# Quantus-Network/qp-zk-circuits

Hardware: AMD Instinct MI355X
Metric: Wormhole proofs/sec (higher is better)
Workload: dtype u64

## Files before the change

qp-zk-circuits_amd/csrc/merkle_kernels_mx.hip:

```cpp
#define POSEIDON_GROUPED_SBOX 1
#include <hip/hip_runtime.h>
#include <vector>
#include "merkle.hpp"
#include "poseidon_mfma.hpp"
#include "prover_kernels.hpp"

using gl::u32;
using gl::u64;

namespace mx {
constexpr int WG = 512;
__constant__ u64 c_poseidon_rc[poseidon::ROUNDS * poseidon::WIDTH];
__device__ uint4 g_table[pmf::TABLE_BYTES / 16];
__device__ uint4 g_table_p2[pmf::TABLE_BYTES / 16];

#define MX_KERNEL __global__ void __launch_bounds__(WG) __attribute__((amdgpu_waves_per_eu(4, 4)))

struct PoseidonV1 {
    static __device__ __forceinline__ const uint4 *table() { return g_table; }
    static __device__ __forceinline__ void permute(u64 (&s)[12], const poseidon2::Params *, const unsigned char *lds) { pmf::permute(s, c_poseidon_rc, lds); }
};
struct Poseidon2QP {
    static __device__ __forceinline__ const uint4 *table() { return g_table_p2; }
    static __device__ __forceinline__ void permute(u64 (&s)[12], const poseidon2::Params *p2, const unsigned char *lds) { pmf::permute_p2qp(s, *p2, lds); }
};
template <class Perm>
__device__ __forceinline__ const unsigned char *table_to_lds() {
    extern __shared__ uint4 mx_lds[];
    const uint4 *t = Perm::table();
    for (int i = threadIdx.x; i < pmf::TABLE_BYTES / 16; i += WG) mx_lds[i] = t[i];
    __syncthreads();
    return (const unsigned char *)mx_lds;
}
__device__ __forceinline__ u32 ilog2_64(u64 x) { return 63u - (u32)__clzll((long long)x); }

template <class Perm>
MX_KERNEL leaf_hash_kernel(MerkleLeafArgs a, const poseidon2::Params *p2) {
    const unsigned char *lds = table_to_lds<Perm>();
    const u64 total = a.n_leaves * a.batch;
    u64 gj = blockIdx.x * (u64)WG + threadIdx.x;
    const bool live = gj < total;
    gj = live ? gj : total - 1;
    const u64 pr = gj >> ilog2_64(a.n_leaves), j = gj & (a.n_leaves - 1);
    a.src0 += pr * a.ps_src0; a.src1 += pr * a.ps_src1; a.digests += pr * a.ps_digests;
    const u32 W = a.ncols0 + a.ncols1;
    auto elem = [&](u32 c) -> u64 {
        return c < a.ncols0 ? a.src0[(u64)c * a.stride0 + j] : a.src1[(u64)(c - a.ncols0) * a.stride1 + j];
    };
    u64 s[12];
#pragma unroll
    for (int i = 0; i < 12; i++) s[i] = 0;
    for (u32 c = 0; c < W; c += 8) {
#pragma unroll
        for (int i = 0; i < 8; i++)
            if (c + i < W) s[i] = elem(c + i);
        Perm::permute(s, p2, lds);
    }
    if (live) {
        u64 *out = a.digests + j * 4;
#pragma unroll
        for (int i = 0; i < 4; i++) out[i] = s[i];
    }
}

template <class Perm>
MX_KERNEL node_kernel(const u64 *in, u64 *out, u64 n_out, u32 batch, u64 ps, u32 per_thread, const poseidon2::Params *p2) {
    const unsigned char *lds = table_to_lds<Perm>();
    const u64 total = n_out * batch;
    const u32 sh = ilog2_64(n_out);
    for (u32 k = 0; k < per_thread; k++) {
        u64 gi = ((u64)blockIdx.x * per_thread + k) * WG + threadIdx.x;
        const bool live = gi < total;
        gi = live ? gi : total - 1;
        const u64 pr = gi >> sh, i = gi & (n_out - 1);
        const ulonglong2 *p = reinterpret_cast<const ulonglong2 *>(in + pr * ps + i * 8);
        const ulonglong2 a = p[0], b = p[1], c = p[2], d = p[3];
        u64 s[12];
        s[0] = a.x; s[1] = a.y; s[2] = b.x; s[3] = b.y; s[4] = c.x; s[5] = c.y; s[6] = d.x; s[7] = d.y;
        s[8] = s[9] = s[10] = s[11] = 0;
        Perm::permute(s, p2, lds);
        if (live) {
            ulonglong2 *o = reinterpret_cast<ulonglong2 *>(out + pr * ps + i * 4);
            o[0] = make_ulonglong2(s[0], s[1]);
            o[1] = make_ulonglong2(s[2], s[3]);
        }
    }
}

template <class Perm>
MX_KERNEL pow_kernel(PowArgs a, const poseidon2::Params *p2) {
    const u32 chunk = blockIdx.x / a.batch, pr = (blockIdx.x % a.batch + chunk) % a.batch;
    const u64 first = (u64)chunk * WG;
    if (first >= a.count) return;
    const u64 base = a.bases[pr];
    if (base == ~0ull) return;
    __shared__ u32 s_leave;
    if (threadIdx.x == 0) s_leave = __hip_atomic_load(&a.results[pr], __ATOMIC_RELAXED, __HIP_MEMORY_SCOPE_AGENT) < base + first ? 1u : 0u;
    __syncthreads();
    if (s_leave) return;
    const unsigned char *lds = table_to_lds<Perm>();
    const u64 idx = first + threadIdx.x, nonce = base + idx;
    const u64 *st = a.states + 12 * (u64)pr;
    u64 s[12];
#pragma unroll
    for (int i = 0; i < 12; i++) s[i] = (i == (int)a.pos) ? nonce : st[i];
    Perm::permute(s, p2, lds);
    if (idx < a.count && (s[7] >> (64 - a.pow_bits)) == 0) atomicMin((unsigned long long *)&a.results[pr], (unsigned long long)nonce);
}

template <class Perm>
MX_KERNEL selftest_kernel(u64 *states, const poseidon2::Params *p2) {
    const unsigned char *lds = table_to_lds<Perm>();
    const u64 t = blockIdx.x * (u64)WG + threadIdx.x;
    u64 s[12];
#pragma unroll
    for (int i = 0; i < 12; i++) s[i] = states[t * 12 + i];
    Perm::permute(s, p2, lds);
#pragma unroll
    for (int i = 0; i < 12; i++) states[t * 12 + i] = s[i];
}
}

template <class Perm>
static hipError_t allow_table_in_lds() {
    hipError_t e = hipFuncSetAttribute((const void *)mx::leaf_hash_kernel<Perm>, hipFuncAttributeMaxDynamicSharedMemorySize, pmf::TABLE_BYTES);
    if (e == hipSuccess) e = hipFuncSetAttribute((const void *)mx::node_kernel<Perm>, hipFuncAttributeMaxDynamicSharedMemorySize, pmf::TABLE_BYTES);
    if (e == hipSuccess) e = hipFuncSetAttribute((const void *)mx::pow_kernel<Perm>, hipFuncAttributeMaxDynamicSharedMemorySize, pmf::TABLE_BYTES);
    return e;
}
template <class Perm, class HostPerm>
static hipError_t device_selftest(HostPerm host_perm, const poseidon2::Params *host_p2) {
    constexpr int N = 4 * mx::WG;
    std::vector<u64> in((size_t)N * 12), out((size_t)N * 12);
    u64 seed = 0x9E3779B97F4A7C15ull;
    for (int t = 0; t < N; t++)
        for (int i = 0; i < 12; i++) {
            seed = seed * 6364136223846793005ull + 1442695040888963407ull;
            u64 v = (seed ^ (seed >> 31)) % gl::P;
            if (t % 9 == 0) v = (i & 1) ? gl::P - 1 - (v & 3) : (v & 7);
            in[(size_t)t * 12 + i] = v;
        }
    u64 *d = nullptr; poseidon2::Params *dp = nullptr; hipStream_t st = nullptr;
    hipError_t e = hipMalloc((void **)&d, in.size() * 8);
    if (e == hipSuccess && host_p2) { e = hipMalloc((void **)&dp, sizeof *host_p2); if (e == hipSuccess) e = hipMemcpy(dp, host_p2, sizeof *host_p2, hipMemcpyHostToDevice); }
    if (e == hipSuccess) e = hipMemcpy(d, in.data(), in.size() * 8, hipMemcpyHostToDevice);
    if (e == hipSuccess) e = hipStreamCreateWithFlags(&st, hipStreamNonBlocking);
    if (e == hipSuccess) e = hipFuncSetAttribute((const void *)mx::selftest_kernel<Perm>, hipFuncAttributeMaxDynamicSharedMemorySize, pmf::TABLE_BYTES);
    if (e == hipSuccess) {
        hipLaunchKernelGGL(mx::selftest_kernel<Perm>, dim3(N / mx::WG), dim3(mx::WG), pmf::TABLE_BYTES, st, d, dp);
        e = hipGetLastError();
        if (e == hipSuccess) e = hipStreamSynchronize(st);
    }
    if (e == hipSuccess) e = hipMemcpy(out.data(), d, out.size() * 8, hipMemcpyDeviceToHost);
    if (e == hipSuccess)
        for (int t = 0; t < N && e == hipSuccess; t++) {
            u64 s[12];
            for (int i = 0; i < 12; i++) s[i] = in[(size_t)t * 12 + i];
            host_perm(s);
            for (int i = 0; i < 12; i++) if (s[i] != out[(size_t)t * 12 + i]) e = hipErrorAssert;
        }
    constexpr u64 NL = 1ull << 19, NN = NL / 2, POW_COUNT = 1ull << 18;
    constexpr u32 WCOLS = 5, POW_BITS = 11, POW_BATCH = 2;
    u64 *d_cols = nullptr, *d_dig = nullptr, *d_pow = nullptr;
    std::vector<u64> cols((size_t)WCOLS * NL), dig(4 * (NL + NN)), powbuf(12 * POW_BATCH + 2 * POW_BATCH);
    if (e == hipSuccess) {
        for (size_t i = 0; i < cols.size(); i++) { seed = seed * 6364136223846793005ull + 1442695040888963407ull; cols[i] = (seed ^ (seed >> 29)) % gl::P; }
        for (u32 b = 0; b < POW_BATCH; b++) {
            for (int i = 0; i < 12; i++) { seed = seed * 6364136223846793005ull + 1442695040888963407ull; powbuf[12 * b + i] = (seed ^ (seed >> 29)) % gl::P; }
            powbuf[12 * POW_BATCH + b] = 1000 * (b + 1);
            powbuf[12 * POW_BATCH + POW_BATCH + b] = ~0ull;
        }
        e = hipMalloc((void **)&d_cols, cols.size() * 8);
        if (e == hipSuccess) e = hipMalloc((void **)&d_dig, dig.size() * 8);
        if (e == hipSuccess) e = hipMalloc((void **)&d_pow, powbuf.size() * 8);
        if (e == hipSuccess) e = hipMemcpy(d_cols, cols.data(), cols.size() * 8, hipMemcpyHostToDevice);
        if (e == hipSuccess) e = hipMemcpy(d_pow, powbuf.data(), powbuf.size() * 8, hipMemcpyHostToDevice);
    }
    if (e == hipSuccess) {
        MerkleLeafArgs la{};
        la.src0 = d_cols; la.stride0 = NL; la.ncols0 = WCOLS; la.n_leaves = NL; la.digests = d_dig; la.batch = 1;
        hipLaunchKernelGGL(mx::leaf_hash_kernel<Perm>, dim3((unsigned)(NL / mx::WG)), dim3(mx::WG), pmf::TABLE_BYTES, st, la, dp);
        hipLaunchKernelGGL(mx::node_kernel<Perm>, dim3((unsigned)(NN / mx::WG)), dim3(mx::WG), pmf::TABLE_BYTES, st, d_dig, d_dig + 4 * NL, NN, 1u, (u64)0, 1u, dp);
        PowArgs pa{};
        pa.states = d_pow; pa.bases = d_pow + 12 * POW_BATCH; pa.results = d_pow + 12 * POW_BATCH + POW_BATCH;
        pa.pos = 3; pa.pow_bits = POW_BITS; pa.batch = POW_BATCH; pa.count = POW_COUNT;
        hipLaunchKernelGGL(mx::pow_kernel<Perm>, dim3((unsigned)(POW_COUNT / mx::WG * POW_BATCH)), dim3(mx::WG), pmf::TABLE_BYTES, st, pa, dp);
        e = hipGetLastError();
        if (e == hipSuccess) e = hipStreamSynchronize(st);
        if (e == hipSuccess) e = hipMemcpy(dig.data(), d_dig, dig.size() * 8, hipMemcpyDeviceToHost);
        if (e == hipSuccess) e = hipMemcpy(powbuf.data(), d_pow, powbuf.size() * 8, hipMemcpyDeviceToHost);
    }
    if (e == hipSuccess) {
        for (u64 w = 0; w < NL / 64 && e == hipSuccess; w++) {
            const u64 j = w * 64 + (w * 7) % 64;
            u64 s[12] = {0};
            for (u32 c = 0; c < WCOLS; c++) s[c] = cols[(size_t)c * NL + j];
            host_perm(s);
            for (int i = 0; i < 4; i++) if (s[i] != dig[4 * j + i]) e = hipErrorAssert;
        }
        for (u64 w = 0; w < NN / 64 && e == hipSuccess; w++) {
            const u64 i0 = w * 64 + (w * 11) % 64;
            u64 s[12] = {0};
            for (int i = 0; i < 8; i++) s[i] = dig[8 * i0 + i];
            host_perm(s);
            for (int i = 0; i < 4; i++) if (s[i] != dig[4 * NL + 4 * i0 + i]) e = hipErrorAssert;
        }
        for (u32 b = 0; b < POW_BATCH && e == hipSuccess; b++) {
            const u64 base = 1000 * (b + 1), got = powbuf[12 * POW_BATCH + POW_BATCH + b];
            u64 want = ~0ull;
            for (u64 k = 0; k < POW_COUNT && want == ~0ull; k++) {
                u64 s[12];
                for (int i = 0; i < 12; i++) s[i] = i == 3 ? base + k : powbuf[12 * b + i];
                host_perm(s);
                if ((s[7] >> (64 - POW_BITS)) == 0) want = base + k;
            }
            if (got != want) e = hipErrorAssert;
        }
    }
    if (d_cols) (void)hipFree(d_cols);
    if (d_dig) (void)hipFree(d_dig);
    if (d_pow) (void)hipFree(d_pow);
    if (st) (void)hipStreamDestroy(st);
    if (d) (void)hipFree(d);
    if (dp) (void)hipFree(dp);
    return e;
}
hipError_t merkle_mx_upload_constants(const u64 *rc360) {
    std::vector<unsigned char> tab(pmf::TABLE_BYTES);
    if (!pmf::build_tables(rc360, tab.data()) || !pmf::host_selfcheck(rc360, tab.data(), 64)) return hipErrorInvalidValue;
    hipError_t e = hipMemcpyToSymbol(HIP_SYMBOL(mx::c_poseidon_rc), rc360, sizeof(u64) * poseidon::ROUNDS * poseidon::WIDTH);
    if (e != hipSuccess) return e;
    e = hipMemcpyToSymbol(HIP_SYMBOL(mx::g_table), tab.data(), pmf::TABLE_BYTES);
    if (e == hipSuccess) e = allow_table_in_lds<mx::PoseidonV1>();
    return e != hipSuccess ? e : device_selftest<mx::PoseidonV1>([&](u64 (&s)[12]) { poseidon::permute(s, rc360); }, nullptr);
}
hipError_t merkle_upload_p2_tables(const poseidon2::Params &qp) {
    std::vector<unsigned char> tab(pmf::TABLE_BYTES);
    if (!pmf::build_tables_p2(qp, tab.data()) || !pmf::host_selfcheck_p2(qp, tab.data(), 64)) return hipErrorInvalidValue;
    hipError_t e = hipMemcpyToSymbol(HIP_SYMBOL(mx::g_table_p2), tab.data(), pmf::TABLE_BYTES);
    if (e == hipSuccess) e = allow_table_in_lds<mx::Poseidon2QP>();
    return e != hipSuccess ? e : device_selftest<mx::Poseidon2QP>([&](u64 (&s)[12]) { poseidon2::permute(s, qp); }, &qp);
}
hipError_t merkle_mx_leaves(const MerkleLeafArgs &a, u64 total, const HasherDev &h, hipStream_t st) {
    const u64 blocks = (total + mx::WG - 1) / mx::WG;
    if (blocks > 0x7FFFFFFFull) return hipErrorInvalidValue;
    if (h.kind == hasher::POSEIDON2) hipLaunchKernelGGL(mx::leaf_hash_kernel<mx::Poseidon2QP>, dim3((unsigned)blocks), dim3(mx::WG), pmf::TABLE_BYTES, st, a, h.p2);
    else hipLaunchKernelGGL(mx::leaf_hash_kernel<mx::PoseidonV1>, dim3((unsigned)blocks), dim3(mx::WG), pmf::TABLE_BYTES, st, a, h.p2);
    return hipGetLastError();
}
hipError_t merkle_mx_nodes(const u64 *in, u64 *out, u64 n_out, u32 batch, u64 ps, const HasherDev &h, hipStream_t st) {
// ... 17 lines not shown
```

qp-zk-circuits_amd/csrc/poseidon.hpp:

```cpp
#pragma once
#include <stddef.h>
#include "gl64.hpp"

namespace poseidon {
using gl::u32;
using gl::u64;

constexpr int WIDTH = 12, RATE = 8, HALF_FULL = 4, PARTIAL = 22, ROUNDS = 30;

GL_HD u64 sbox7(u64 x) {
    u64 x2 = gl::sqr(x), x4 = gl::sqr(x2), x3 = gl::mul(x, x2);
    return gl::mul(x3, x4);
}
#if defined(__HIP_DEVICE_COMPILE__) && defined(POSEIDON_GROUPED_SBOX)
template <int N>
__device__ __forceinline__ void sbox7_layer(u64 (&x)[N]) {
    u64 x2[N], x3[N], x4[N];
    gl::mul_group(x2, x, x);
    gl::mul_group(x4, x2, x2);
    gl::mul_group(x3, x, x2);
    gl::mul_group(x, x3, x4);
}
__device__ __forceinline__ u64 sbox7_lane(u64 x) {
    u64 a[1] = {x}, x2[1];
// ... 14 lines not shown
}
GL_HD u64 sbox7_lane(u64 x) { return sbox7(x); }
#endif

GL_HD void mds_layer_naive(u64 (&s)[WIDTH]) {
    constexpr u32 C[WIDTH] = {17, 15, 41, 16, 2, 28, 13, 13, 39, 18, 34, 20};
    u32 lo[WIDTH], hi[WIDTH];
#pragma unroll
    for (int i = 0; i < WIDTH; i++) { lo[i] = (u32)s[i]; hi[i] = (u32)(s[i] >> 32); }
#pragma unroll
    for (int r = 0; r < WIDTH; r++) {
        u64 al = 0, ah = 0;
#pragma unroll
        for (int i = 0; i < WIDTH; i++) {
            const int j = (i + r) % WIDTH;
            al += (u64)lo[j] * C[i];
            ah += (u64)hi[j] * C[i];
        }
        if (r == 0) { al += (u64)lo[0] * 8u; ah += (u64)hi[0] * 8u; }
        u64 low = al + (ah << 32);
        u32 top = (u32)(ah >> 32) + (low < al ? 1u : 0u);
        s[r] = gl::reduce96(low, top);
    }
}

typedef long long i64;
GL_HD i64 shl(i64 x, int k) { return (i64)((u64)x << k); }
GL_HD void mds_circulant_half(const i64 (&x)[WIDTH], i64 (&o)[WIDTH]) {
    i64 U1[3], Um[3], F[3], H[3];
#pragma unroll
    for (int b = 0; b < 3; b++) {
        const i64 e = x[b] + x[b + 6], f = x[b] - x[b + 6], g = x[b + 3] + x[b + 9], h = x[b + 3] - x[b + 9];
        U1[b] = e + g; Um[b] = e - g; F[b] = f; H[b] = h;
    }
    const i64 T = U1[0] + U1[1] + U1[2];
    const i64 A[3] = {T + U1[2], T + U1[0], T + U1[1]};
    const i64 B[3] = {shl(Um[2], 3) - Um[0] - shl(Um[1], 1),
                      -(shl(Um[0], 3) + Um[1] + shl(Um[2], 1)),
                      shl(Um[0], 1) - shl(Um[1], 3) - Um[2]};
    const i64 f0 = F[0], f1 = F[1], f2 = F[2], h0 = H[0], h1 = H[1], h2 = H[2];
    const i64 R[3] = {shl(f0, 1) - h0 + f1 - shl(h1, 4) + f2 + shl(h2, 2),
                      -shl(f0, 2) + h0 + shl(f1, 1) - h1 + f2 - shl(h2, 4),
                      shl(f0, 4) + h0 - shl(f1, 2) + h1 + shl(f2, 1) - h2};
    const i64 I[3] = {f0 + shl(h0, 1) + shl(f1, 4) + h1 - shl(f2, 2) + h2,
                      -f0 - shl(h0, 2) + f1 + shl(h1, 1) + shl(f2, 4) + h2,
                      -f0 + shl(h0, 4) - f1 - shl(h1, 2) + f2 + shl(h2, 1)};
#pragma unroll
    for (int b = 0; b < 3; b++) {
        const i64 a16 = shl(A[b], 4), p = a16 + B[b], q = a16 - B[b];
        o[b] = p + R[b]; o[b + 3] = q + I[b]; o[b + 6] = p - R[b]; o[b + 9] = q - I[b];
    }
}

GL_HD void mds_layer(u64 (&s)[WIDTH]) {
    i64 lo[WIDTH], hi[WIDTH], ol[WIDTH], oh[WIDTH];
#pragma unroll
    for (int i = 0; i < WIDTH; i++) { lo[i] = (i64)(u32)s[i]; hi[i] = (i64)(s[i] >> 32); }
    mds_circulant_half(lo, ol);
    mds_circulant_half(hi, oh);
    ol[0] += shl(lo[0], 3); oh[0] += shl(hi[0], 3);
#pragma unroll
    for (int r = 0; r < WIDTH; r++) {
        const u64 al = (u64)ol[r], ah = (u64)oh[r];
        const u64 low = al + (ah << 32);
        const u32 top = (u32)(ah >> 32) + (low < al ? 1u : 0u);
        s[r] = gl::reduce96(low, top);
    }
}

struct Spectrum { i64 U1[3], Um[3], F[3], H[3]; };
GL_HD void spectrum_of(const i64 (&x)[WIDTH], Spectrum &s) {
#pragma unroll
    for (int b = 0; b < 3; b++) {
        const i64 e = x[b] + x[b + 6], g = x[b + 3] + x[b + 9];
        s.U1[b] = e + g; s.Um[b] = e - g; s.F[b] = x[b] - x[b + 6]; s.H[b] = x[b + 3] - x[b + 9];
    }
}
GL_HD void spectrum_times_circulant(Spectrum &s) {
    const i64 T = s.U1[0] + s.U1[1] + s.U1[2];
    const i64 A0 = T + s.U1[2], A1 = T + s.U1[0], A2 = T + s.U1[1];
    const i64 B0 = shl(s.Um[2], 3) - s.Um[0] - shl(s.Um[1], 1);
    const i64 B1 = -(shl(s.Um[0], 3) + s.Um[1] + shl(s.Um[2], 1));
    const i64 B2 = shl(s.Um[0], 1) - shl(s.Um[1], 3) - s.Um[2];
    const i64 f0 = s.F[0], f1 = s.F[1], f2 = s.F[2], h0 = s.H[0], h1 = s.H[1], h2 = s.H[2];
    const i64 R0 = shl(f0, 1) - h0 + f1 - shl(h1, 4) + f2 + shl(h2, 2);
    const i64 R1 = -shl(f0, 2) + h0 + shl(f1, 1) - h1 + f2 - shl(h2, 4);
    const i64 R2 = shl(f0, 4) + h0 - shl(f1, 2) + h1 + shl(f2, 1) - h2;
    const i64 I0 = f0 + shl(h0, 1) + shl(f1, 4) + h1 - shl(f2, 2) + h2;
    const i64 I1 = -f0 - shl(h0, 2) + f1 + shl(h1, 1) + shl(f2, 4) + h2;
    const i64 I2 = -f0 + shl(h0, 4) - f1 - shl(h1, 2) + f2 + shl(h2, 1);
    s.U1[0] = shl(A0, 6); s.U1[1] = shl(A1, 6); s.U1[2] = shl(A2, 6);
    s.Um[0] = shl(B0, 2); s.Um[1] = shl(B1, 2); s.Um[2] = shl(B2, 2);
    s.F[0] = shl(R0, 1); s.F[1] = shl(R1, 1); s.F[2] = shl(R2, 1);
    s.H[0] = shl(I0, 1); s.H[1] = shl(I1, 1); s.H[2] = shl(I2, 1);
}
GL_HD i64 spectrum_lane0(const Spectrum &s) { return (s.U1[0] + s.Um[0] + shl(s.F[0], 1)) >> 2; }
GL_HD void vector_of(const Spectrum &s, i64 (&x)[WIDTH]) {
#pragma unroll
    for (int b = 0; b < 3; b++) {
        const i64 p = s.U1[b] + s.Um[b], q = s.U1[b] - s.Um[b], f2 = shl(s.F[b], 1), h2 = shl(s.H[b], 1);
        x[b] = (p + f2) >> 2; x[b + 6] = (p - f2) >> 2; x[b + 3] = (q + h2) >> 2; x[b + 9] = (q - h2) >> 2;
    }
}
GL_HD u64 join_halves(i64 lo, i64 hi) {
    const u64 al = (u64)lo, ah = (u64)hi;
    const u64 low = al + (ah << 32);
    const u32 top = (u32)(ah >> 32) + (low < al ? 1u : 0u);
    return gl::reduce96(low, top);
}
GL_HD void renormalize_pair(i64 &lo, i64 &hi) {
    const i64 k = (lo >> 32) & ~(i64)3;
    lo -= shl(k, 32); hi += k;
    const i64 m = (hi >> 32) & ~(i64)3;
    hi -= shl(m, 32); hi += m; lo -= m;
}
GL_HD void renormalize(Spectrum &sl, Spectrum &sh) {
#pragma unroll
    for (int b = 0; b < 3; b++) {
        renormalize_pair(sl.U1[b], sh.U1[b]); renormalize_pair(sl.Um[b], sh.Um[b]);
        renormalize_pair(sl.F[b], sh.F[b]); renormalize_pair(sl.H[b], sh.H[b]);
    }
// ... 238 lines not shown
```

qp-zk-circuits_amd/csrc/poseidon_mfma.hpp:

```cpp
#pragma once
#include <string.h>
#include <utility>
#include "poseidon.hpp"

namespace pmf {
using gl::u32;
using gl::u64;
#if defined(__HIPCC__)
typedef int v4i __attribute__((ext_vector_type(4)));
typedef int v16i __attribute__((ext_vector_type(16)));
#endif

constexpr int LIMBS = 8, N_GROUP = 6, N_FIN = 3, FIN_STEPS = 9, N_ELEM = 36;
constexpr int group_steps(int g) { return 3 + g; }
constexpr int group_base(int g) { int b = 0; for (int i = 0; i < g; i++) b += group_steps(i); return b; }
constexpr int N_GROUP_TILES = group_base(N_GROUP);
constexpr int N_TILES = N_GROUP_TILES + N_FIN * FIN_STEPS;
constexpr int CINIT_OFF = N_TILES * 1024;
constexpr int G_OFF = CINIT_OFF + (N_GROUP + N_FIN) * 128;
constexpr int TABLE_BYTES = G_OFF + 32;
static_assert(N_GROUP_TILES == 33 && TABLE_BYTES % 16 == 0, "table layout");
constexpr u64 DIGIT_BIAS = 0x8080808080808080ull;

constexpr u64 mds_entry(int r, int j) {
    constexpr u32 C[12] = {17, 15, 41, 16, 2, 28, 13, 13, 39, 18, 34, 20};
    return C[(j - r + 12) % 12] + ((r == 0 && j == 0) ? 8 : 0);
}
constexpr u64 small_g(int d) {
    u64 R[12] = {1, 0, 0, 0, 0, 0, 0, 0, 0, 0, 0, 0};
    for (int it = 0; it < d; it++) {
        u64 T[12] = {};
        for (int j = 1; j < 12; j++)
            for (int i = 0; i < 12; i++) T[j] += R[i] * mds_entry(i, j);
        for (int j = 0; j < 12; j++) R[j] = T[j];
    }
    u64 g = 0;
    for (int i = 0; i < 12; i++) g += R[i] * mds_entry(i, 0);
    return g;
}
constexpr u32 G0 = (u32)small_g(0), G1 = (u32)small_g(1), G2 = (u32)small_g(2);
static_assert(small_g(0) == 25 && small_g(2) < (1ull << 32), "group coefficients fit one word");

GL_HD u64 to_digits(u64 v) {
    u64 t = v + DIGIT_BIAS;
    t += (t < v) ? 0xFFFFFFFFull : 0ull;
    return t ^ DIGIT_BIAS;
}
GL_HD u32 byte_perm(u32 s0, u32 s1, u32 sel) {
#if defined(__HIP_DEVICE_COMPILE__)
    return __builtin_amdgcn_perm(s0, s1, sel);
#else
    const u64 pool = ((u64)s0 << 32) | s1;
    u32 r = 0;
    for (int i = 0; i < 4; i++) r |= (u32)((pool >> (8 * ((sel >> (8 * i)) & 7))) & 0xFF) << (8 * i);
    return r;
#endif
}
GL_HD u64 recombine(const u32 (&z)[LIMBS]) {
    const u32 a0 = (z[3] << 24) | z[0], a1 = byte_perm(z[6], z[3], 0x05040201u), a2 = z[6] >> 16;
    const u32 b0 = z[1] << 8, b1 = (z[7] << 24) | z[4], b2 = z[7] >> 8;
    const u32 c0 = z[2] << 16, c1 = byte_perm(z[5], z[2], 0x06050402u);
    typedef unsigned __int128 u128;
    const u128 A = ((u128)a2 << 64) | ((u128)a1 << 32) | a0;
    const u128 B = ((u128)b2 << 64) | ((u128)b1 << 32) | b0;
    const u128 Cc = ((u128)c1 << 32) | c0;
    const u128 S = A + B + Cc;
    return gl::reduce96((u64)S, (u32)(S >> 64));
}
GL_HD u64 mul_small(u64 y, u32 g) {
    const u64 p0 = (u64)(u32)y * g;
    const u64 p1 = (u64)(u32)(y >> 32) * g + (p0 >> 32);
    return gl::reduce96((p1 << 32) | (u32)p0, (u32)(p1 >> 32));
}
constexpr int row_of(int output, int limb) { const int i = 8 * (output & 1) + limb; return (i & 3) + 8 * (i >> 2) + 4 * (output >> 1); }

#if !defined(__HIP_DEVICE_COMPILE__)
namespace host {
typedef unsigned __int128 u128;
inline u64 fmul(u64 a, u64 b) { return (u64)((u128)a * b % gl::P); }
inline u64 fadd(u64 a, u64 b) { return (u64)(((u128)a + b) % gl::P); }
inline u64 fsub(u64 a, u64 b) { return (u64)(((u128)a + gl::P - b % gl::P) % gl::P); }
inline bool const_digits(u64 w, signed char (&d)[LIMBS]) {
    w %= gl::P;
    __int128 rep = w <= 0x7F7F7F7F7F7F7F7Full ? (__int128)w : (__int128)w - (__int128)gl::P;
    for (int a = 0; a < LIMBS; a++) {
        int dg = (int)(rep & 255);
        if (dg >= 128) dg -= 256;
        d[a] = (signed char)dg;
        rep = (rep - dg) / 256;
    }
    return rep == 0;
}
struct Rows { u64 w[4][N_ELEM]; u64 addc[4]; };
inline bool fill_tiles(const Rows &rw, int steps, unsigned char *tiles, unsigned char *cinit) {
    static signed char dig[4][N_ELEM][8][LIMBS];
    for (int o = 0; o < 4; o++)
        for (int e = 0; e < N_ELEM; e++) {
            u64 w = rw.w[o][e] % gl::P;
            for (int b = 0; b < 8; b++) { if (!const_digits(w, dig[o][e][b])) return false; w = fmul(w, 256); }
        }
    for (int q = 0; q < steps; q++)
        for (int o = 0; o < 4; o++)
            for (int limb = 0; limb < LIMBS; limb++)
                for (int k = 0; k < 32; k++) {
                    const int lane = row_of(o, limb) + 32 * (k >> 4), j = k & 15, e = 4 * q + (k >> 3), b = k & 7;
                    tiles[(size_t)q * 1024 + lane * 16 + j] = (unsigned char)dig[o][e][b][limb];
                }
    u64 bias = 0, pw = 1u << 23;
    for (int l = 0; l < LIMBS; l++) { bias = fadd(bias, pw); pw = fmul(pw, 256); }
    for (int h = 0; h < 2; h++)
        for (int i = 0; i < 16; i++) {
            const u64 c = fsub(rw.addc[2 * h + (i >> 3)], bias);
            const u32 v = (1u << 23) + (u32)((c >> (8 * (i & 7))) & 0xFF);
            memcpy(cinit + h * 64 + i * 4, &v, 4);
        }
    return true;
}
struct Linear {
    u64 M[12][12], pre[12][12];
    u64 rc[22][12], after[12];
};
inline bool build_tables(const Linear &L, unsigned char *tab) {
    static u64 R[23][12], G[22], Q[22][12], NP[12][12];
    const auto &M = L.M;
    for (int j = 0; j < 12; j++) R[0][j] = j == 0;
// ... 45 lines not shown
inline bool build_tables(const u64 *rc, unsigned char *tab) {
    static Linear L;
    memset(&L, 0, sizeof L);
    for (int r = 0; r < 12; r++) for (int j = 0; j < 12; j++) L.M[r][j] = L.pre[r][j] = mds_entry(r, j);
    for (int k = 0; k < 22; k++) L.rc[k][0] = rc[(4 + k) * 12];
    for (int i = 1; i < 12; i++) L.rc[0][i] = rc[4 * 12 + i];
    for (int i = 0; i < 12; i++) L.after[i] = rc[26 * 12 + i];
    if (!build_tables(L, tab)) return false;
    u64 g[3]; memcpy(g, tab + G_OFF, sizeof g);
    return g[0] == G0 && g[1] == G1 && g[2] == G2;
}
inline bool build_tables_gate(const u64 *rcp, unsigned char *tab) {
    static Linear L;
    memset(&L, 0, sizeof L);
    for (int r = 0; r < 12; r++) for (int j = 0; j < 12; j++) L.M[r][j] = L.pre[r][j] = mds_entry(r, j);
    for (int k = 0; k < 22; k++) for (int i = 0; i < 12; i++) L.rc[k][i] = rcp[(4 + k) * 12 + i];
    for (int i = 0; i < 12; i++) L.after[i] = rcp[26 * 12 + i];
    return build_tables(L, tab);
}
inline bool build_tables_p2(const poseidon2::Params &p, unsigned char *tab) {
    static Linear L;
    memset(&L, 0, sizeof L);
    for (int j = 0; j < 12; j++) {
        u64 e[12] = {}, f[12] = {};
        e[j] = f[j] = 1;
        poseidon2::int_layer(e, p); poseidon2::ext_layer_qp(f);
        for (int i = 0; i < 12; i++) { L.M[i][j] = gl::canon(e[i]); L.pre[i][j] = gl::canon(f[i]); }
    }
    for (int k = 0; k < 22; k++) L.rc[k][0] = p.rc_int[k];
    for (int i = 0; i < 12; i++) L.after[i] = p.rc_ext[4 * 12 + i];
    return build_tables(L, tab);
}
inline bool emu_gemm(const unsigned char *tab, int tile0, int cidx, int steps, const u64 *D, u32 (&Z)[4][LIMBS]) {
    for (int o = 0; o < 4; o++)
        for (int limb = 0; limb < LIMBS; limb++) {
            const int row = row_of(o, limb);
            u32 c; memcpy(&c, tab + CINIT_OFF + cidx * 128 + (o >> 1) * 64 + (8 * (o & 1) + limb) * 4, 4);
            long long acc = c;
            for (int q = 0; q < steps; q++)
                for (int k = 0; k < 32; k++) {
                    const int lane = row + 32 * (k >> 4), j = k & 15;
                    const int a = (signed char)tab[(size_t)(tile0 + q) * 1024 + lane * 16 + j];
                    const int bdig = (signed char)(D[4 * q + (k >> 3)] >> (8 * (k & 7)));
                    acc += (long long)a * bdig;
                }
            if (acc < 0 || acc >= (1 << 24)) return false;
            Z[o][limb] = (u32)acc;
        }
    return true;
}
inline bool emu_partial_rounds(u64 (&s)[12], const unsigned char *tab) {
    u64 D[N_ELEM] = {}, y[24], G[3];
    memcpy(G, tab + G_OFF, sizeof G);
    for (int e = 0; e < 12; e++) D[e] = to_digits(s[e]);
    for (int g = 0; g < N_GROUP; g++) {
        u32 Z[4][LIMBS];
        if (!emu_gemm(tab, group_base(g), g, group_steps(g), D, Z)) return false;
        for (int o = 0; o < 4 && 4 * g + o < 22; o++) {
            const int k = 4 * g + o;
            u64 x = recombine(Z[o]);
            for (int j = 4 * g; j < k; j++) x = gl::add(x, G[k - 1 - j] >> 32 ? gl::mul(y[j], G[k - 1 - j]) : mul_small(y[j], (u32)G[k - 1 - j]));
            y[k] = poseidon::sbox7_lane(x);
        }
        for (int o = 0; o < 4 && 4 * g + o < 22; o++) D[12 + 4 * g + o] = to_digits(y[4 * g + o]);
    }
    for (int f = 0; f < N_FIN; f++) {
        u32 Z[4][LIMBS];
        if (!emu_gemm(tab, N_GROUP_TILES + f * FIN_STEPS, N_GROUP + f, FIN_STEPS, D, Z)) return false;
        for (int o = 0; o < 4; o++) s[4 * f + o] = recombine(Z[o]);
    }
    return true;
}
inline bool emu_permute_textbook(u64 (&s)[12], const u64 *rcp, const unsigned char *tab) {
    using namespace poseidon;
    int r = 0;
    for (int k = 0; k < HALF_FULL; k++, r++) {
        for (int i = 0; i < WIDTH; i++) s[i] = sbox7(gl::add_canonical(s[i], rcp[r * WIDTH + i]));
        if (k + 1 < HALF_FULL) mds_layer(s);
    }
    if (!emu_partial_rounds(s, tab)) return false;
    r += 1 + PARTIAL;
    for (int i = 0; i < WIDTH; i++) s[i] = sbox7(s[i]);
    mds_layer(s);
    for (int k = 1; k < HALF_FULL; k++, r++) {
        for (int i = 0; i < WIDTH; i++) s[i] = sbox7(gl::add_canonical(s[i], rcp[r * WIDTH + i]));
        mds_layer(s);
    }
    for (int i = 0; i < WIDTH; i++) s[i] = gl::canon(s[i]);
    return true;
}
inline bool emu_permute(u64 (&s)[12], const u64 *rc, const unsigned char *tab) {
    using namespace poseidon;
    int r = 0;
    for (int k = 0; k < HALF_FULL; k++, r++) {
        for (int i = 0; i < WIDTH; i++) s[i] = gl::add_canonical(s[i], rc[r * WIDTH + i]);
        sbox7_layer(s);
        if (k + 1 < HALF_FULL) mds_layer(s);
    }
    if (!emu_partial_rounds(s, tab)) return false;
    r += 1 + PARTIAL;
    sbox7_layer(s); mds_layer(s);
    for (int k = 1; k < HALF_FULL; k++, r++) {
        for (int i = 0; i < WIDTH; i++) s[i] = gl::add_canonical(s[i], rc[r * WIDTH + i]);
        sbox7_layer(s);
        mds_layer(s);
    }
    for (int i = 0; i < WIDTH; i++) s[i] = gl::canon(s[i]);
    return true;
}
inline bool emu_permute_p2(u64 (&s)[12], const poseidon2::Params &p, const unsigned char *tab) {
    poseidon2::ext_layer_qp(s);
    for (int r = 0; r < 4; r++) {
        for (int i = 0; i < 12; i++) s[i] = gl::add(s[i], p.rc_ext[r * 12 + i]);
        poseidon::sbox7_layer(s);
// ... 58 lines not shown
    auto r = __builtin_amdgcn_permlane32_swap(x, y, false, false);
    x = r[0]; y = r[1];
}
struct Run {
    u32 Dlo[N_ELEM], Dhi[N_ELEM];
    v4i B0[FIN_STEPS], B1[FIN_STEPS];
    u64 y[24];
    u64 Gd[3];
    const unsigned char *lds;
};
__device__ __forceinline__ void form_step(Run &st, int q) {
    swap32(st.Dlo[4 * q], st.Dlo[4 * q + 2]); swap32(st.Dhi[4 * q], st.Dhi[4 * q + 2]);
    swap32(st.Dlo[4 * q + 1], st.Dlo[4 * q + 3]); swap32(st.Dhi[4 * q + 1], st.Dhi[4 * q + 3]);
    st.B0[q] = v4i{(int)st.Dlo[4 * q], (int)st.Dhi[4 * q], (int)st.Dlo[4 * q + 1], (int)st.Dhi[4 * q + 1]};
    st.B1[q] = v4i{(int)st.Dlo[4 * q + 2], (int)st.Dhi[4 * q + 2], (int)st.Dlo[4 * q + 3], (int)st.Dhi[4 * q + 3]};
}
template <int STEPS>
__device__ __forceinline__ void gemm(const Run &st, int tile0, int cidx, u32 (&Z)[4][LIMBS]) {
    const int lane = threadIdx.x & 63;
    const v4i *cp = (const v4i *)(st.lds + CINIT_OFF + cidx * 128 + (lane >> 5) * 64);
    v16i a0, a1;
#pragma unroll
    for (int i = 0; i < 4; i++) {
        const v4i c = cp[i];
        a0[4 * i] = c[0]; a0[4 * i + 1] = c[1]; a0[4 * i + 2] = c[2]; a0[4 * i + 3] = c[3];
    }
    a1 = a0;
    const v4i *ap = (const v4i *)(st.lds + (size_t)tile0 * 1024) + lane;
#pragma unroll
    for (int q = 0; q < STEPS; q++) {
        const v4i a = ap[q * 64];
        a0 = __builtin_amdgcn_mfma_i32_32x32x32_i8(a, st.B0[q], a0, 0, 0, 0);
        a1 = __builtin_amdgcn_mfma_i32_32x32x32_i8(a, st.B1[q], a1, 0, 0, 0);
    }
#ifndef PMF_NO_KEEPALIVE
    asm volatile("" : "+v"(a0), "+v"(a1));
#endif
#pragma unroll
    for (int i = 0; i < 16; i++) {
        u32 x = (u32)a0[i], yv = (u32)a1[i];
        swap32(x, yv);
        Z[i >> 3][i & 7] = x; Z[2 + (i >> 3)][i & 7] = yv;
    }
}
struct SboxOfInput { __device__ __forceinline__ u64 operator()(int, u64 x) const { return poseidon::sbox7_lane(x); } };
template <int G, bool SMALL_G, class F>
__device__ __forceinline__ void group_step(Run &st, F &f) {
    u32 Z[4][LIMBS];
    gemm<group_steps(G)>(st, group_base(G), G, Z);
    constexpr int n = 4 * G + 4 <= 22 ? 4 : 22 - 4 * G;
#pragma unroll
    for (int o = 0; o < n; o++) {
        const int k = 4 * G + o;
        u64 x = recombine(Z[o]);
        constexpr u32 Gc[3] = {G0, G1, G2};
#pragma unroll
        for (int j = 4 * G; j < k; j++) x = gl::add(x, SMALL_G ? mul_small(st.y[j], Gc[k - 1 - j]) : gl::mul(st.y[j], st.Gd[k - 1 - j]));
        st.y[k] = f(k, x);
    }
#pragma unroll
    for (int o = 0; o < n; o++) {
        const u64 t = to_digits(st.y[4 * G + o]);
        st.Dlo[12 + 4 * G + o] = (u32)t; st.Dhi[12 + 4 * G + o] = (u32)(t >> 32);
    }
    form_step(st, 3 + G);
}
template <bool SMALL_G, class F, int... G>
__device__ __forceinline__ void all_groups(Run &st, F &f, std::integer_sequence<int, G...>) { (group_step<G, SMALL_G>(st, f), ...); }

template <bool SMALL_G, class F>
__device__ __forceinline__ void partial_rounds(u64 (&s)[12], const unsigned char *lds, F &f) {
    Run st;
    st.lds = lds;
    if (!SMALL_G) {
#pragma unroll
        for (int d = 0; d < 3; d++) {
            const u64 g = *(const u64 *)(lds + G_OFF + 8 * d);
            st.Gd[d] = ((u64)(u32)__builtin_amdgcn_readfirstlane((int)(g >> 32)) << 32) | (u32)__builtin_amdgcn_readfirstlane((int)(u32)g);
        }
    }
#pragma unroll
    for (int e = 0; e < N_ELEM; e++) {
        const u64 t = e < 12 ? to_digits(s[e]) : 0;
        st.Dlo[e] = (u32)t; st.Dhi[e] = (u32)(t >> 32);
    }
    form_step(st, 0); form_step(st, 1); form_step(st, 2);
    all_groups<SMALL_G>(st, f, std::make_integer_sequence<int, N_GROUP>{});
#pragma unroll
    for (int f = 0; f < N_FIN; f++) {
        u32 Z[4][LIMBS];
        gemm<FIN_STEPS>(st, N_GROUP_TILES + f * FIN_STEPS, N_GROUP + f, Z);
#pragma unroll
        for (int o = 0; o < 4; o++) s[4 * f + o] = recombine(Z[o]);
    }
}
__device__ __forceinline__ void permute_head(u64 (&s)[12], const u64 *rc, const unsigned char *lds) {
    using namespace poseidon;
    int r = 0;
    for (int k = 0; k < HALF_FULL; k++, r++) {
#pragma unroll
        for (int i = 0; i < WIDTH; i++) s[i] = gl::add_canonical(s[i], rc[r * WIDTH + i]);
        sbox7_layer(s);
        if (k + 1 < HALF_FULL) mds_layer(s);
    }
    SboxOfInput f;
    partial_rounds<true>(s, lds, f);
}
__device__ __forceinline__ void permute_tail(u64 (&s)[12], const u64 *rc) {
    using namespace poseidon;
    int r = HALF_FULL + 1 + PARTIAL;
    sbox7_layer(s);
    mds_layer(s);
    for (int k = 1; k < HALF_FULL; k++, r++) {
#pragma unroll
        for (int i = 0; i < WIDTH; i++) s[i] = gl::add_canonical(s[i], rc[r * WIDTH + i]);
        sbox7_layer(s);
        mds_layer(s);
    }
#pragma unroll
    for (int i = 0; i < WIDTH; i++) s[i] = gl::canon(s[i]);
}
__device__ __forceinline__ void permute(u64 (&s)[12], const u64 *rc, const unsigned char *lds) {
    permute_head(s, rc, lds);
    permute_tail(s, rc);
}
__device__ __forceinline__ void permute_p2qp(u64 (&s)[12], const poseidon2::Params &p, const unsigned char *lds) {
    poseidon2::ext_layer_qp(s);
    for (int r = 0; r < 4; r++) {
#pragma unroll
        for (int i = 0; i < 12; i++) s[i] = gl::add_canonical(s[i], p.rc_ext[r * 12 + i]);
        poseidon::sbox7_layer(s);
        if (r < 3) poseidon2::ext_layer_qp(s);
    }
    SboxOfInput f;
    partial_rounds<false>(s, lds, f);
    poseidon::sbox7_layer(s);
    poseidon2::ext_layer_qp(s);
    for (int r = 5; r < 8; r++) {
#pragma unroll
        for (int i = 0; i < 12; i++) s[i] = gl::add_canonical(s[i], p.rc_ext[r * 12 + i]);
        poseidon::sbox7_layer(s);
        poseidon2::ext_layer_qp(s);
    }
#pragma unroll
    for (int i = 0; i < 12; i++) s[i] = gl::canon(s[i]);
}
#elif defined(__HIPCC__)
__device__ void permute(u64 (&s)[12], const u64 *rc, const unsigned char *lds);
__device__ void permute_head(u64 (&s)[12], const u64 *rc, const unsigned char *lds);
__device__ void permute_tail(u64 (&s)[12], const u64 *rc);
__device__ void permute_p2qp(u64 (&s)[12], const poseidon2::Params &p, const unsigned char *lds);
template <bool SMALL_G, class F> __device__ void partial_rounds(u64 (&)[12], const unsigned char *, F &) {}
#endif

}
```

Baseline: 1470.

## Compute only needed output rows of final MDS layer and fuse small-G reductions

Splits the Poseidon V1 permutation so the final MDS layer is evaluated only for the state rows the caller consumes: digest rows in node and leaf hashing, one row for PoW, and rate or capacity rows depending on how many leaf columns remain. It also replaces per-term reduce-and-add of small group coefficients in the partial rounds with a single wide accumulation followed by one reduce96. The tail round loop is rearranged so the last sbox is separate from its MDS. This cuts redundant modular reductions and dead output rows, at the cost of more template specialisation, an asm barrier to keep state copies, and a tighter coefficient bound.

```diff
diff --git a/qp-zk-circuits_amd/csrc/merkle_kernels_mx.hip b/qp-zk-circuits_amd/csrc/merkle_kernels_mx.hip
--- a/qp-zk-circuits_amd/csrc/merkle_kernels_mx.hip
+++ b/qp-zk-circuits_amd/csrc/merkle_kernels_mx.hip
@@ -18,12 +18,29 @@
 
 struct PoseidonV1 {
     static __device__ __forceinline__ const uint4 *table() { return g_table; }
-    static __device__ __forceinline__ void permute(u64 (&s)[12], const poseidon2::Params *, const unsigned char *lds) { pmf::permute(s, c_poseidon_rc, lds); }
+    static __device__ __forceinline__ void body(u64 (&s)[12], const poseidon2::Params *, const unsigned char *lds) {
+        pmf::permute_head(s, c_poseidon_rc, lds);
+        pmf::permute_tail_rounds(s, c_poseidon_rc);
+    }
+    template <int FIRST, int COUNT, bool CANON>
+    static __device__ __forceinline__ void last_rows(u64 (&s)[12]) { pmf::last_layer_rows<FIRST, COUNT, CANON>(s); }
+    static __device__ __forceinline__ void own_copy(u64 (&s)[12]) {
+#pragma unroll
+        for (int i = 0; i < 12; i++) asm volatile("" : "+v"(s[i]));
+    }
 };
 struct Poseidon2QP {
     static __device__ __forceinline__ const uint4 *table() { return g_table_p2; }
-    static __device__ __forceinline__ void permute(u64 (&s)[12], const poseidon2::Params *p2, const unsigned char *lds) { pmf::permute_p2qp(s, *p2, lds); }
+    static __device__ __forceinline__ void body(u64 (&s)[12], const poseidon2::Params *p2, const unsigned char *lds) { pmf::permute_p2qp(s, *p2, lds); }
+    template <int FIRST, int COUNT, bool CANON>
+    static __device__ __forceinline__ void last_rows(u64 (&)[12]) {}
+    static __device__ __forceinline__ void own_copy(u64 (&)[12]) {}
 };
+template <class Perm, int FIRST, int COUNT, bool CANON>
+__device__ __forceinline__ void permute_rows(u64 (&s)[12], const poseidon2::Params *p2, const unsigned char *lds) {
+    Perm::body(s, p2, lds);
+    Perm::template last_rows<FIRST, COUNT, CANON>(s);
+}
 template <class Perm>
 __device__ __forceinline__ const unsigned char *table_to_lds() {
     extern __shared__ uint4 mx_lds[];
@@ -54,7 +71,11 @@
 #pragma unroll
         for (int i = 0; i < 8; i++)
             if (c + i < W) s[i] = elem(c + i);
-        Perm::permute(s, p2, lds);
+        Perm::body(s, p2, lds);
+        const u32 rest = W - c;
+        if (rest <= 8) { Perm::own_copy(s); Perm::template last_rows<0, 4, true>(s); }
+        else if (rest >= 16) { Perm::own_copy(s); Perm::template last_rows<8, 4, false>(s); }
+        else { Perm::own_copy(s); Perm::template last_rows<0, 12, false>(s); }
     }
     if (live) {
         u64 *out = a.digests + j * 4;
@@ -78,7 +99,7 @@
         u64 s[12];
         s[0] = a.x; s[1] = a.y; s[2] = b.x; s[3] = b.y; s[4] = c.x; s[5] = c.y; s[6] = d.x; s[7] = d.y;
         s[8] = s[9] = s[10] = s[11] = 0;
-        Perm::permute(s, p2, lds);
+        permute_rows<Perm, 0, 4, true>(s, p2, lds);
         if (live) {
             ulonglong2 *o = reinterpret_cast<ulonglong2 *>(out + pr * ps + i * 4);
             o[0] = make_ulonglong2(s[0], s[1]);
@@ -104,7 +125,7 @@
     u64 s[12];
 #pragma unroll
     for (int i = 0; i < 12; i++) s[i] = (i == (int)a.pos) ? nonce : st[i];
-    Perm::permute(s, p2, lds);
+    permute_rows<Perm, 7, 1, true>(s, p2, lds);
     if (idx < a.count && (s[7] >> (64 - a.pow_bits)) == 0) atomicMin((unsigned long long *)&a.results[pr], (unsigned long long)nonce);
 }
 
@@ -115,7 +136,7 @@
     u64 s[12];
 #pragma unroll
     for (int i = 0; i < 12; i++) s[i] = states[t * 12 + i];
-    Perm::permute(s, p2, lds);
+    permute_rows<Perm, 0, 12, true>(s, p2, lds);
 #pragma unroll
     for (int i = 0; i < 12; i++) states[t * 12 + i] = s[i];
 }
@@ -160,7 +181,7 @@
             for (int i = 0; i < 12; i++) if (s[i] != out[(size_t)t * 12 + i]) e = hipErrorAssert;
         }
     constexpr u64 NL = 1ull << 19, NN = NL / 2, POW_COUNT = 1ull << 18;
-    constexpr u32 WCOLS = 5, POW_BITS = 11, POW_BATCH = 2;
+    constexpr u32 WCOLS = 17, POW_BITS = 11, POW_BATCH = 2;
     u64 *d_cols = nullptr, *d_dig = nullptr, *d_pow = nullptr;
     std::vector<u64> cols((size_t)WCOLS * NL), dig(4 * (NL + NN)), powbuf(12 * POW_BATCH + 2 * POW_BATCH);
     if (e == hipSuccess) {
@@ -194,8 +215,10 @@
         for (u64 w = 0; w < NL / 64 && e == hipSuccess; w++) {
             const u64 j = w * 64 + (w * 7) % 64;
             u64 s[12] = {0};
-            for (u32 c = 0; c < WCOLS; c++) s[c] = cols[(size_t)c * NL + j];
-            host_perm(s);
+            for (u32 c = 0; c < WCOLS; c += 8) {
+                for (u32 i = 0; i < 8 && c + i < WCOLS; i++) s[i] = cols[(size_t)(c + i) * NL + j];
+                host_perm(s);
+            }
             for (int i = 0; i < 4; i++) if (s[i] != dig[4 * j + i]) e = hipErrorAssert;
         }
         for (u64 w = 0; w < NN / 64 && e == hipSuccess; w++) {
diff --git a/qp-zk-circuits_amd/csrc/poseidon.hpp b/qp-zk-circuits_amd/csrc/poseidon.hpp
--- a/qp-zk-circuits_amd/csrc/poseidon.hpp
+++ b/qp-zk-circuits_amd/csrc/poseidon.hpp
@@ -90,7 +90,9 @@
     }
 }
 
-GL_HD void mds_layer(u64 (&s)[WIDTH]) {
+template <int FIRST, int COUNT>
+GL_HD void mds_layer_rows(u64 (&s)[WIDTH]) {
+    static_assert(FIRST >= 0 && COUNT >= 1 && FIRST + COUNT <= WIDTH, "rows of the state");
     i64 lo[WIDTH], hi[WIDTH], ol[WIDTH], oh[WIDTH];
 #pragma unroll
     for (int i = 0; i < WIDTH; i++) { lo[i] = (i64)(u32)s[i]; hi[i] = (i64)(s[i] >> 32); }
@@ -98,13 +100,14 @@
     mds_circulant_half(hi, oh);
     ol[0] += shl(lo[0], 3); oh[0] += shl(hi[0], 3);
 #pragma unroll
-    for (int r = 0; r < WIDTH; r++) {
+    for (int r = FIRST; r < FIRST + COUNT; r++) {
         const u64 al = (u64)ol[r], ah = (u64)oh[r];
         const u64 low = al + (ah << 32);
         const u32 top = (u32)(ah >> 32) + (low < al ? 1u : 0u);
         s[r] = gl::reduce96(low, top);
     }
 }
+GL_HD void mds_layer(u64 (&s)[WIDTH]) { mds_layer_rows<0, WIDTH>(s); }
 
 struct Spectrum { i64 U1[3], Um[3], F[3], H[3]; };
 GL_HD void spectrum_of(const i64 (&x)[WIDTH], Spectrum &s) {
diff --git a/qp-zk-circuits_amd/csrc/poseidon_mfma.hpp b/qp-zk-circuits_amd/csrc/poseidon_mfma.hpp
--- a/qp-zk-circuits_amd/csrc/poseidon_mfma.hpp
+++ b/qp-zk-circuits_amd/csrc/poseidon_mfma.hpp
@@ -39,7 +39,7 @@
     return g;
 }
 constexpr u32 G0 = (u32)small_g(0), G1 = (u32)small_g(1), G2 = (u32)small_g(2);
-static_assert(small_g(0) == 25 && small_g(2) < (1ull << 32), "group coefficients fit one word");
+static_assert(small_g(0) == 25 && small_g(1) < small_g(2) && small_g(2) < (1ull << 21), "group coefficients: the bound of reduce96_terms");
 
 GL_HD u64 to_digits(u64 v) {
     u64 t = v + DIGIT_BIAS;
@@ -56,7 +56,7 @@
     return r;
 #endif
 }
-GL_HD u64 recombine(const u32 (&z)[LIMBS]) {
+GL_HD void recombine_wide(const u32 (&z)[LIMBS], u64 &lo, u32 &top) {
     const u32 a0 = (z[3] << 24) | z[0], a1 = byte_perm(z[6], z[3], 0x05040201u), a2 = z[6] >> 16;
     const u32 b0 = z[1] << 8, b1 = (z[7] << 24) | z[4], b2 = z[7] >> 8;
     const u32 c0 = z[2] << 16, c1 = byte_perm(z[5], z[2], 0x06050402u);
@@ -65,12 +65,23 @@
     const u128 B = ((u128)b2 << 64) | ((u128)b1 << 32) | b0;
     const u128 Cc = ((u128)c1 << 32) | c0;
     const u128 S = A + B + Cc;
-    return gl::reduce96((u64)S, (u32)(S >> 64));
-}
-GL_HD u64 mul_small(u64 y, u32 g) {
-    const u64 p0 = (u64)(u32)y * g;
-    const u64 p1 = (u64)(u32)(y >> 32) * g + (p0 >> 32);
-    return gl::reduce96((p1 << 32) | (u32)p0, (u32)(p1 >> 32));
+    lo = (u64)S; top = (u32)(S >> 64);
+}
+GL_HD u64 recombine(const u32 (&z)[LIMBS]) {
+    u64 lo; u32 top;
+    recombine_wide(z, lo, top);
+    return gl::reduce96(lo, top);
+}
+constexpr int MAX_GROUP_TERMS = 3;
+GL_HD u64 reduce96_terms(u64 lo, u32 top, const u64 *y, const u32 *g, int n) {
+    if (n == 0) return gl::reduce96(lo, top);
+    u64 al = (u32)lo, ah = ((u64)top << 32) | (lo >> 32);
+#if defined(__HIP_DEVICE_COMPILE__)
+#pragma unroll
+#endif
+    for (int i = 0; i < n; i++) { al += (u64)(u32)y[i] * g[i]; ah += (y[i] >> 32) * g[i]; }
+    const u64 low = al + (ah << 32);
+    return gl::reduce96(low, (u32)(ah >> 32) + (low < al ? 1u : 0u));
 }
 constexpr int row_of(int output, int limb) { const int i = 8 * (output & 1) + limb; return (i & 3) + 8 * (i >> 2) + 4 * (output >> 1); }
 
@@ -222,14 +233,23 @@
 inline bool emu_partial_rounds(u64 (&s)[12], const unsigned char *tab) {
     u64 D[N_ELEM] = {}, y[24], G[3];
     memcpy(G, tab + G_OFF, sizeof G);
+    const bool small = G[0] == G0 && G[1] == G1 && G[2] == G2;
     for (int e = 0; e < 12; e++) D[e] = to_digits(s[e]);
     for (int g = 0; g < N_GROUP; g++) {
         u32 Z[4][LIMBS];
         if (!emu_gemm(tab, group_base(g), g, group_steps(g), D, Z)) return false;
         for (int o = 0; o < 4 && 4 * g + o < 22; o++) {
             const int k = 4 * g + o;
-            u64 x = recombine(Z[o]);
-            for (int j = 4 * g; j < k; j++) x = gl::add(x, G[k - 1 - j] >> 32 ? gl::mul(y[j], G[k - 1 - j]) : mul_small(y[j], (u32)G[k - 1 - j]));
+            u64 x;
+            if (small) {
+                u64 lo; u32 top, gg[MAX_GROUP_TERMS];
+                recombine_wide(Z[o], lo, top);
+                for (int i = 0; i < o; i++) gg[i] = (u32)G[o - 1 - i];
+                x = reduce96_terms(lo, top, y + 4 * g, gg, o);
+            } else {
+                x = recombine(Z[o]);
+                for (int j = 4 * g; j < k; j++) x = gl::add(x, gl::mul(y[j], G[k - 1 - j]));
+            }
             y[k] = poseidon::sbox7_lane(x);
         }
         for (int o = 0; o < 4 && 4 * g + o < 22; o++) D[12 + 4 * g + o] = to_digits(y[4 * g + o]);
@@ -394,10 +414,20 @@
 #pragma unroll
     for (int o = 0; o < n; o++) {
         const int k = 4 * G + o;
-        u64 x = recombine(Z[o]);
-        constexpr u32 Gc[3] = {G0, G1, G2};
-#pragma unroll
-        for (int j = 4 * G; j < k; j++) x = gl::add(x, SMALL_G ? mul_small(st.y[j], Gc[k - 1 - j]) : gl::mul(st.y[j], st.Gd[k - 1 - j]));
+        u64 x;
+        if constexpr (SMALL_G) {
+            constexpr u32 Gc[3] = {G0, G1, G2};
+            u64 lo, yy[MAX_GROUP_TERMS] = {};
+            u32 top, gg[MAX_GROUP_TERMS] = {};
+            recombine_wide(Z[o], lo, top);
+#pragma unroll
+            for (int i = 0; i < o; i++) { yy[i] = st.y[4 * G + i]; gg[i] = Gc[o - 1 - i]; }
+            x = reduce96_terms(lo, top, yy, gg, o);
+        } else {
+            x = recombine(Z[o]);
+#pragma unroll
+            for (int j = 4 * G; j < k; j++) x = gl::add(x, gl::mul(st.y[j], st.Gd[k - 1 - j]));
+        }
         st.y[k] = f(k, x);
     }
 #pragma unroll
@@ -448,20 +478,31 @@
     SboxOfInput f;
     partial_rounds<true>(s, lds, f);
 }
-__device__ __forceinline__ void permute_tail(u64 (&s)[12], const u64 *rc) {
+__device__ __forceinline__ void permute_tail_rounds(u64 (&s)[12], const u64 *rc) {
     using namespace poseidon;
     int r = HALF_FULL + 1 + PARTIAL;
-    sbox7_layer(s);
-    mds_layer(s);
     for (int k = 1; k < HALF_FULL; k++, r++) {
-#pragma unroll
-        for (int i = 0; i < WIDTH; i++) s[i] = gl::add_canonical(s[i], rc[r * WIDTH + i]);
         sbox7_layer(s);
         mds_layer(s);
-    }
-#pragma unroll
-    for (int i = 0; i < WIDTH; i++) s[i] = gl::canon(s[i]);
-}
+#pragma unroll
+        for (int i = 0; i < WIDTH; i++) s[i] = gl::add_canonical(s[i], rc[r * WIDTH + i]);
+    }
+    sbox7_layer(s);
+}
+template <int FIRST, int COUNT, bool CANON>
+__device__ __forceinline__ void last_layer_rows(u64 (&s)[12]) {
+    poseidon::mds_layer_rows<FIRST, COUNT>(s);
+    if (CANON) {
+#pragma unroll
+        for (int i = FIRST; i < FIRST + COUNT; i++) s[i] = gl::canon(s[i]);
+    }
+}
+template <int FIRST, int COUNT, bool CANON>
+__device__ __forceinline__ void permute_tail_rows(u64 (&s)[12], const u64 *rc) {
+    permute_tail_rounds(s, rc);
+    last_layer_rows<FIRST, COUNT, CANON>(s);
+}
+__device__ __forceinline__ void permute_tail(u64 (&s)[12], const u64 *rc) { permute_tail_rows<0, 12, true>(s, rc); }
 __device__ __forceinline__ void permute(u64 (&s)[12], const u64 *rc, const unsigned char *lds) {
     permute_head(s, rc, lds);
     permute_tail(s, rc);
@@ -491,6 +532,9 @@
 __device__ void permute(u64 (&s)[12], const u64 *rc, const unsigned char *lds);
 __device__ void permute_head(u64 (&s)[12], const u64 *rc, const unsigned char *lds);
 __device__ void permute_tail(u64 (&s)[12], const u64 *rc);
+__device__ void permute_tail_rounds(u64 (&s)[12], const u64 *rc);
+template <int FIRST, int COUNT, bool CANON> __device__ void last_layer_rows(u64 (&)[12]) {}
+template <int FIRST, int COUNT, bool CANON> __device__ void permute_tail_rows(u64 (&)[12], const u64 *) {}
 __device__ void permute_p2qp(u64 (&s)[12], const poseidon2::Params &p, const unsigned char *lds);
 template <bool SMALL_G, class F> __device__ void partial_rounds(u64 (&)[12], const unsigned char *, F &) {}
 #endif
```

Result: faster. 1510, median of 6 (+2.7%).
